# awkrail/svpc

Hardware: AMD Instinct MI355X
Metric: train steps/sec (vivt, batch=16, clip_seq=12) (higher is better)
Workload: dtype bf16x3

## Files before the change

### include/svpc_hip.h

```cpp
#ifndef SVPC_HIP_H
#define SVPC_HIP_H
#include <stddef.h>
#ifdef __cplusplus
extern "C" {
#endif

typedef struct ihipStream_t* svpc_stream_t;
typedef unsigned long long svpc_u64;

#define SVPC_ACT_NONE 0
#define SVPC_ACT_RELU 1
#define SVPC_ACT_GELU 2
#define SVPC_ACT_SIGMOID 3

const char* svpc_last_error(void);
int svpc_abi_version(void);

int svpc_ln_fwd(const float* x, const int* src_rows, const float* res, const float* gamma, const float* beta, float* y,
                float* mean, float* rstd, int R, int D, float eps, float p_pre, unsigned site_pre, float p_post,
                unsigned site_post, const svpc_u64* seed, const float* add1, int mod1, const float* add2, const int* idx2,
                svpc_stream_t stream);
int svpc_ln_fwd_t(const void* x, int x_dt, const int* src_rows, const void* res, const float* gamma, const float* beta, void* y,
                  int y_dt, float* mean, float* rstd, int R, int D, float eps, float p_pre, unsigned site_pre, float p_post,
                  unsigned site_post, const svpc_u64* seed, const float* add1, int mod1, const float* add2, const int* idx2,
// ... 8 lines not shown
int svpc_ln_param_grads(const float* partial, int R, int D, float* dgamma, float* dbeta, int accumulate, svpc_stream_t stream);
int svpc_ln_fwd_s(const void* x, int x_dt, int ldx, int lox, const int* src_rows, const void* res, int ldr, int lor, const float* gamma,
                  const float* beta, void* y, int y_dt, int ldy, int loy, float* mean, float* rstd, int R, int D, float eps, float p_pre,
                  unsigned site_pre, float p_post, unsigned site_post, const svpc_u64* seed, const float* add1, int mod1,
                  const float* add2, const int* idx2, svpc_stream_t stream);
int svpc_ln_bwd_rows_s(const void* dy, const void* x, int x_dt, int ldx, int y_dt, const int* src_rows, const void* res, int ldr,
                       const float* gamma, const float* mean, const float* rstd, void* dh, void* dx, float* partial, int R, int D,
                       float p_pre, unsigned site_pre, float p_post, unsigned site_post, const svpc_u64* seed, svpc_stream_t stream);
int svpc_bucket_colsum_t(const void* x, int x_dt, int ldx, const int* idx, int R, int C, int K, float* out, int accumulate,
                         float* workspace, svpc_stream_t stream);
typedef struct svpc_finalize_entry { const float* partial; float* out0; float* out1; int groups, ncols, split; } svpc_finalize_entry;
int svpc_colsum_partial_t(const void* x, int x_dt, int ldx, int R, int C, float* partial, svpc_stream_t stream);
typedef struct svpc_colsum_entry { const void* x; float* partial; int dt, ldx, R, C; } svpc_colsum_entry;
int svpc_multi_colsum(const svpc_colsum_entry* entries, int n, svpc_stream_t stream);
int svpc_multi_finalize_max(void);
int svpc_multi_finalize(const svpc_finalize_entry* entries, int n, svpc_stream_t stream);
int svpc_ln_bwd_groups(int R);
int svpc_ln_param_only_groups(int R);
int svpc_ln_param_grads_g(const float* partial, int groups, int D, float* dgamma, float* dbeta, int accumulate, svpc_stream_t stream);
int svpc_ln_bwd(const float* dy, const float* x, const int* src_rows, const float* res, const float* gamma,
                const float* mean, const float* rstd, float* dh, float* dx, float* dgamma, float* dbeta, int accumulate,
                float* workspace, int R, int D, float p_pre, unsigned site_pre, float p_post, unsigned site_post,
                const svpc_u64* seed, svpc_stream_t stream);
int svpc_colsum_chunks(int R);
int svpc_bucket_colsum(const float* x, int ldx, const int* idx, int R, int C, int K, float* out, int accumulate,
                       float* workspace, svpc_stream_t stream);

int svpc_gemm_f32(const float* A, int lda, int a_kc, const float* B, int ldb, int b_kc, float* C, int ldc, float* Z, int M, int N,
                  int K, const float* bias, int act, float p_drop, unsigned site, const svpc_u64* seed, int accumulate,
                  float* workspace, size_t workspace_bytes, svpc_stream_t stream);
int svpc_gemm_bf16(const float* A, int lda, int a_kc, const float* B, int ldb, int b_kc, float* C, int ldc, float* Z, int M, int N,
                   int K, const float* bias, int act, float p_drop, unsigned site, const svpc_u64* seed, int accumulate,
                   float* workspace, size_t workspace_bytes, svpc_stream_t stream);
int svpc_gemm_mx(const void* A, int a_dt, int lda, int a_kc, const void* B, int b_dt, int ldb, int b_kc, void* C, int c_dt, int ldc,
                 void* Z, int M, int N, int K, const float* bias, int act, float p_drop, unsigned site, const svpc_u64* seed,
                 int accumulate, float* workspace, size_t workspace_bytes, svpc_stream_t stream);
int svpc_gemm_glds_supported(int a_kc, int b_kc, int lda, int ldb, int M, int N, int K);
int svpc_gemm_glds(const void* A, int lda, int a_kc, const void* B, int ldb, int b_kc, void* C, int c_dt, int ldc, void* Z, int M, int N,
                   int K, const float* bias, int act, float p_drop, unsigned site, const svpc_u64* seed, int accumulate,
                   float* workspace, size_t workspace_bytes, svpc_stream_t stream);
int svpc_gemm_glds_r(const void* A, int lda, int a_kc, const void* B, int ldb, int b_kc, void* C, int c_dt, int ldc, void* Z, const void* R,
                     int M, int N, int K, const float* bias, int act, float p_drop, unsigned site, const svpc_u64* seed, int accumulate,
                     float* workspace, size_t workspace_bytes, svpc_stream_t stream);
int svpc_gemm_glds_rg(const void* A, int lda, int a_kc, const void* B, int ldb, int b_kc, void* C, int c_dt, int ldc, void* Z, const void* R,
                      const void* G, int gact, int M, int N, int K, const float* bias, int act, float p_drop, unsigned site,
                      const svpc_u64* seed, int accumulate, float* workspace, size_t workspace_bytes, svpc_stream_t stream);
int svpc_gemm_p8(const void* A, int lda, const void* B, int ldb, void* C, int ldc, void* Z, int M, int N, int K, const float* bias, int act,
                 svpc_stream_t stream);
int svpc_gemm_p8x3_supported(int lda, int a_lo, int ldb, int ldc, int c_lo, int ldz, int M, int N, int K);
int svpc_gemm_p8x3(const void* A, int lda, int a_lo, const void* B, int ldb, long long b_lo, void* C, int ldc, int c_lo, void* Z, int ldz,
                   int M, int N, int K, const float* bias, int act, svpc_stream_t stream);
int svpc_gemm_s4x3(const void* A, int lda, int a_lo, const void* B, int ldb, long long b_lo, void* C, int ldc, int c_lo, void* Z, int ldz,
                   int M, int N, int K, const float* bias, int act, svpc_stream_t stream);
int svpc_gemm_s4t_supported(int lda, int ldb, int ldc, int M, int N, int K);
int svpc_gemm_s4t(const void* A, int lda, const void* B, int ldb, void* C, int ldc, const void* R, int M, int N, int K, svpc_stream_t stream);
int svpc_gemm_p8t_supported(int lda, int ldb, int ldc, int M, int N, int K);
int svpc_gemm_p8t(const void* A, int lda, const void* B, int ldb, void* C, int ldc, const void* G, int gact, const void* R, int M, int N, int K,
                  svpc_stream_t stream);
int svpc_gemm_l32_supported(int a_kc, int b_kc, int lda, int ldb, int M, int N, int K);
int svpc_gemm_l32_preferred(int a_kc, int b_kc, int lda, int ldb, int M, int N, int K);
int svpc_gemm_l32(const float* A, int lda, int a_kc, const float* B, int ldb, int b_kc, float* C, int ldc, float* Z, int M, int N, int K,
                  const float* bias, int act, float p_drop, unsigned site, const svpc_u64* seed, int accumulate, float* workspace,
                  size_t workspace_bytes, svpc_stream_t stream);
int svpc_gemm_l32_r(const float* A, int lda, int a_kc, const float* B, int ldb, int b_kc, float* C, int ldc, float* Z, const float* R, int M,
                    int N, int K, const float* bias, int act, float p_drop, unsigned site, const svpc_u64* seed, int accumulate,
                    float* workspace, size_t workspace_bytes, svpc_stream_t stream);
int svpc_gemm_l32_rg(const float* A, int lda, int a_kc, const float* B, int ldb, int b_kc, float* C, int ldc, const float* R, const float* G,
                     int gact, int M, int N, int K, int accumulate, float* workspace, size_t workspace_bytes, svpc_stream_t stream);
int svpc_gemm_l32_x3(const float* A, int lda, int a_kc, const float* B, int ldb, int b_kc, float* C, int ldc, float* Z, const float* R, int M,
                     int N, int K, const float* bias, int act, float p_drop, unsigned site, const svpc_u64* seed, int accumulate,
                     float* workspace, size_t workspace_bytes, svpc_stream_t stream);
typedef struct svpc_gemm_problem { const float* A; const float* B; float* C; int M, N, K, lda, ldb, ldc; } svpc_gemm_problem;
int svpc_gemm_group(const svpc_gemm_problem* problems, int n, int a_kc, int b_kc, int accumulate, svpc_stream_t stream);
int svpc_gemm_group_x3(const svpc_gemm_problem* problems, int n, int a_kc, int b_kc, int accumulate, svpc_stream_t stream);
typedef struct svpc_wgrad_problem {
    const float* dz; const float* x; float* dw; float* db;
    int n_out, n_in, rows, ld_dz, ld_x, ld_dw;
} svpc_wgrad_problem;
int svpc_gemm_group_wgrad_max(void);
int svpc_gemm_group_wgrad_bf16_p8_ok(const void* problems, int n);
int svpc_gemm_group_wgrad_bf16_p8(const void* problems, int n, float* workspace, size_t workspace_bytes, svpc_stream_t stream);
int svpc_gemm_group_wgrad_bf16(const svpc_wgrad_problem* problems, int n, svpc_stream_t stream);
int svpc_gemm_group_wgrad_bf16_ws(const svpc_wgrad_problem* problems, int n, float* workspace, size_t workspace_bytes,
                                  svpc_stream_t stream);
int svpc_gemm_group_wgrad(const svpc_wgrad_problem* problems, int n, svpc_stream_t stream);
int svpc_act_bwd(const float* dy, const float* aux, float* dz, size_t n, int act, float p, unsigned site, const svpc_u64* seed,
                 svpc_stream_t stream);

int svpc_act_bwd_t(const void* dy, const void* aux, void* dz, int dt, size_t n, int act, float p, unsigned site, const svpc_u64* seed,
                   svpc_stream_t stream);

int svpc_attn_fwd(const float* Q, int ldq, const float* K, int ldk, const float* V, int ldv, float* O, int ldo, float* LSE,
                  const int* seq, int n_seq, int H, int dh, int max_q, int max_k, const float* key_mask, int causal, float scale,
                  float p_drop, unsigned site, const svpc_u64* seed, svpc_stream_t stream);
int svpc_attn_q1_fwd(const float* Q, int ldq, const float* K, int ldk, const float* V, int ldv, float* O, int ldo, float* LSE,
                     const int* seq, int n_seq, int H, int dh, int max_k, const float* key_mask, float scale, svpc_stream_t stream);
int svpc_attn_q1_ln_supported(int D, int dh, int n_keys, int ldq, int ldkv, int ldnew, int ldx, int ldo);
int svpc_attn_q1_ln_fwd(const float* Q, int ldq, float* K, float* V, int ldkv, int k_stride, int n_keys, const float* newK, const float* newV,
                        int ldnew, const float* X, int ldx, const float* gamma, const float* beta, float eps, float* O, int ldo, int T, int D,
                        int dh, float scale, svpc_stream_t stream);
int svpc_attn_q1_ln_idx_fwd(const float* Q, int ldq, float* K, float* V, int ldkv, int k_stride, int n_keys, const int* key_rows, int ld_rows,
                            int q_group, const float* newK, const float* newV, int ldnew, const float* X, int ldx, const float* gamma,
                            const float* beta, float eps, float* O, int ldo, int T, int D, int dh, float scale, svpc_stream_t stream);
int svpc_attn_bwd(const float* Q, int ldq, const float* K, int ldk, const float* V, int ldv, const float* O, int ldo,
                  const float* LSE, const float* dO, int lddo, float* dQ, int lddq, float* dK, int lddk, float* dV, int lddv,
                  float* delta, const int* seq, int n_seq, int H, int dh, int max_q, int max_k, const float* key_mask, int causal,
                  float scale, float p_drop, unsigned site, const svpc_u64* seed, svpc_stream_t stream);

// ... 202 lines not shown
```

### svpc_amd/csrc/gemm_common.h

```cpp
#pragma once
#include "common.h"

typedef float floatx16 __attribute__((ext_vector_type(16)));

struct Epi {
    const float* bias; int act; float p_drop; uint32_t site; const u64* seed; int accumulate;
    float* Z;
    const void* R;
    const void* G; int gact;
};

__device__ __forceinline__ void epilogue_store(float v, int row, int col, float* __restrict__ C, int ldc, const Epi& e,
                                               u64 seed, float inv_keep) {
    if (e.bias) v += e.bias[col];
    const size_t o = (size_t)row * ldc + col;
    if (e.Z) e.Z[o] = v;
    v = apply_act(v, e.act);
    if (e.p_drop > 0.f) v *= drop_scale(seed, e.site, o, e.p_drop, inv_keep);
    if (e.G) v *= act_grad_from_aux(reinterpret_cast<const float*>(e.G)[o], e.gact, false);
    if (e.accumulate) v += C[o];
    if (e.R) v += reinterpret_cast<const float*>(e.R)[o];
    C[o] = v;
}

// ... 67 lines not shown
    return (xcd < r ? xcd * (q + 1) : r * (q + 1) + (xcd - r) * q) + (orig >> 3);
}


template <typename TC>
__global__ __launch_bounds__(256) void splitk_reduce1_kernel(const float* __restrict__ slabs, int splitk, TC* __restrict__ C, int ldc,
                                                             int M, int N, Epi epi) {
    const size_t i = (size_t)blockIdx.x * 256 + threadIdx.x;
    if (i >= (size_t)M * N) return;
    const int row = (int)(i / N), col = (int)(i - (size_t)row * N);
    float s = 0.f;
    for (int k = 0; k < splitk; ++k) s += slabs[(size_t)k * M * N + i];
    const u64 seed = epi.p_drop > 0.f ? epi.seed[0] : 0ull;
    const float inv_keep = epi.p_drop > 0.f ? 1.0f / (1.0f - epi.p_drop) : 1.0f;
    epilogue_store_t<TC>(s, row, col, C, ldc, epi, seed, inv_keep);
}
template <typename TC>
__global__ __launch_bounds__(256) void splitk_reduce4_kernel(const float* __restrict__ slabs, int splitk, TC* __restrict__ C, int ldc,
                                                             int M, int N, Epi epi) {
    const size_t q = (size_t)blockIdx.x * 256 + threadIdx.x, nq = (size_t)M * N / 4;
    if (q >= nq) return;
    const size_t i = q * 4;
    const int row = (int)(i / N), col = (int)(i - (size_t)row * N);
    const float4* p = reinterpret_cast<const float4*>(slabs) + q;
    float4 s = make_float4(0.f, 0.f, 0.f, 0.f);
    int k = 0;
    for (; k + 4 <= splitk; k += 4) {
        const float4 a = p[(size_t)k * nq], b = p[(size_t)(k + 1) * nq], c = p[(size_t)(k + 2) * nq], d = p[(size_t)(k + 3) * nq];
        s.x += a.x; s.y += a.y; s.z += a.z; s.w += a.w;
        s.x += b.x; s.y += b.y; s.z += b.z; s.w += b.w;
        s.x += c.x; s.y += c.y; s.z += c.z; s.w += c.w;
        s.x += d.x; s.y += d.y; s.z += d.z; s.w += d.w;
    }
    for (; k < splitk; ++k) {
        const float4 a = p[(size_t)k * nq];
        s.x += a.x; s.y += a.y; s.z += a.z; s.w += a.w;
    }
    const u64 seed = epi.p_drop > 0.f ? epi.seed[0] : 0ull;
    const float inv_keep = epi.p_drop > 0.f ? 1.0f / (1.0f - epi.p_drop) : 1.0f;
    epilogue_store_t<TC>(s.x, row, col, C, ldc, epi, seed, inv_keep);
    epilogue_store_t<TC>(s.y, row, col + 1, C, ldc, epi, seed, inv_keep);
    epilogue_store_t<TC>(s.z, row, col + 2, C, ldc, epi, seed, inv_keep);
    epilogue_store_t<TC>(s.w, row, col + 3, C, ldc, epi, seed, inv_keep);
}
template <typename TC>
static inline void launch_splitk_reduce(const float* slabs, int splitk, TC* C, int ldc, int M, int N, const Epi& epi, hipStream_t stream) {
    const size_t n = (size_t)M * N;
    if (N % 4 == 0 && ((((uintptr_t)slabs) & 15) == 0))
        hipLaunchKernelGGL(splitk_reduce4_kernel<TC>, dim3((unsigned)((n / 4 + 255) / 256)), dim3(256), 0, stream, slabs, splitk, C, ldc, M, N,
                           epi);
    else
        hipLaunchKernelGGL(splitk_reduce1_kernel<TC>, dim3((unsigned)((n + 255) / 256)), dim3(256), 0, stream, slabs, splitk, C, ldc, M, N, epi);
}
```

### svpc_amd/csrc/gemm_s4t.hip

```cpp
#include "gemm_common.h"
#include <stdlib.h>

typedef __bf16 bf16x8 __attribute__((ext_vector_type(8)));
typedef float floatx4 __attribute__((ext_vector_type(4)));
typedef short short4s __attribute__((ext_vector_type(4)));
typedef const void __attribute__((address_space(1))) * s4t_gptr;
typedef void __attribute__((address_space(3))) * s4t_lptr;

constexpr int S4T_BK = 64;
constexpr int S4T_HALF = 128 * S4T_BK * 2;
constexpr int S4T_STAGE = 2 * S4T_HALF;

__device__ __forceinline__ bf16x8 s4t_frag_tr(const char* __restrict__ a) {
    typedef short4s __attribute__((address_space(3))) * lds_ptr;
    const short4s lo = __builtin_amdgcn_ds_read_tr16_b64_v4i16((lds_ptr)(a));
    const short4s hi = __builtin_amdgcn_ds_read_tr16_b64_v4i16((lds_ptr)(a + 4 * 256));
    union { short s[8]; bf16x8 v; } u;
    u.s[0] = lo[0]; u.s[1] = lo[1]; u.s[2] = lo[2]; u.s[3] = lo[3];
    u.s[4] = hi[0]; u.s[5] = hi[1]; u.s[6] = hi[2]; u.s[7] = hi[3];
    return u.v;
}

template <bool HASR, int NS>
__global__ __launch_bounds__(512, NS == 2 ? 2 : 1) void gemm_s4t_kernel(const __bf16* __restrict__ A, int lda, const __bf16* __restrict__ B, int ldb,
                                                                        __bf16* __restrict__ C, int ldc, const __bf16* __restrict__ R, int M,
                                                                        int N, int K, int tiles_m, int tiles_n, int remap) {
    __shared__ __attribute__((aligned(1024))) char smem[NS * S4T_STAGE];
    const int wg = remap ? xcd_remap(blockIdx.x, tiles_m * tiles_n) : (int)blockIdx.x;
    const int tm = wg / tiles_n, tn = wg - tm * tiles_n;
    const int m0 = tm * 128, n0 = tn * 128;
    const int nk = K / S4T_BK;
    const int lane = threadIdx.x & 63, wave = __builtin_amdgcn_readfirstlane(threadIdx.x >> 6);
    const int wr = wave >> 1, wc = wave & 1;

    const int sr = lane >> 2, sc = (lane & 3) ^ (((lane >> 5) & 1) << 1);
    const __bf16* const ga = A + (size_t)min(m0 + 16 * wave + sr, M - 1) * lda + 8 * sc;
    const __bf16* gb[2];
#pragma unroll
    for (int u = 0; u < 2; ++u) {
        const int kr = 8 * wave + 4 * u + (lane >> 4);
        const int fx = 2 * ((kr & 3) | ((kr >> 1) & 4));
        const int col = min(n0 + 8 * ((lane & 15) ^ fx), N - 8);
        gb[u] = B + (size_t)kr * ldb + col;
    }
    const size_t stepB = (size_t)S4T_BK * ldb;
#define S4T_ISSUE(t)                                                                                                              \
    do {                                                                                                                          \
        char* st_ = smem + ((t) % NS) * S4T_STAGE;                                                                                \
        const __bf16* sa_ = ga + (size_t)(t) * S4T_BK;                                                                            \
        __builtin_amdgcn_global_load_lds((s4t_gptr)(sa_), (s4t_lptr)(st_ + ((wave * 2) << 10)), 16, 0, 0);                        \
        __builtin_amdgcn_global_load_lds((s4t_gptr)(sa_ + 32), (s4t_lptr)(st_ + ((wave * 2 + 1) << 10)), 16, 0, 0);               \
        __builtin_amdgcn_global_load_lds((s4t_gptr)(gb[0] + (size_t)(t) * stepB), (s4t_lptr)(st_ + S4T_HALF + wave * 2048), 16, 0, 0);        \
        __builtin_amdgcn_global_load_lds((s4t_gptr)(gb[1] + (size_t)(t) * stepB), (s4t_lptr)(st_ + S4T_HALF + wave * 2048 + 1024), 16, 0, 0); \
    } while (0)
    const int fr_off = (lane & 15) * 64 + ((((lane >> 4) ^ (((lane >> 3) & 1) << 1))) << 4);
#define S4T_FRAGA(img, blk, kb) (*reinterpret_cast<const bf16x8*>((img) + (((blk) * 2 + (kb)) << 10) + fr_off))
    const int tg = lane >> 4, tq = (lane & 15) >> 2, tp = lane & 3;
    const int tfx = 2 * (tq + 4 * (tg & 1));
    const int tb_off = (8 * tg + tq) * 256 + ((tp & 1) << 3);
    const int tp1 = tp >> 1;
#define S4T_FRAGB(img, cb, kb) s4t_frag_tr((img) + (kb) * (32 * 256) + tb_off + (((((2 * (cb)) ^ tfx)) | tp1) << 4))

    floatx4 acc[2][4];
#pragma unroll
    for (int i = 0; i < 2; ++i)
#pragma unroll
        for (int j = 0; j < 4; ++j) acc[i][j] = floatx4{0.f, 0.f, 0.f, 0.f};

#pragma unroll
    for (int t = 0; t < NS - 1; ++t)
        if (t < nk) S4T_ISSUE(t);
    for (int t = 0; t < nk; ++t) {
        if (NS == 4 && t + 2 < nk) asm volatile("s_waitcnt vmcnt(8)" ::: "memory");
        else if (NS >= 3 && t + 1 < nk) asm volatile("s_waitcnt vmcnt(4)" ::: "memory");
        else asm volatile("s_waitcnt vmcnt(0)" ::: "memory");
        __builtin_amdgcn_s_barrier();
        __builtin_amdgcn_sched_barrier(0);
        if (t + NS - 1 < nk) S4T_ISSUE(t + NS - 1);
        const char* sa = smem + (t % NS) * S4T_STAGE;
        const char* sb = sa + S4T_HALF;
#pragma unroll
        for (int kb = 0; kb < 2; ++kb) {
            bf16x8 bfr[4], afr[2];
#pragma unroll
            for (int j = 0; j < 4; ++j) bfr[j] = S4T_FRAGB(sb, wc * 4 + j, kb);
#pragma unroll
            for (int i = 0; i < 2; ++i) afr[i] = S4T_FRAGA(sa, wr * 2 + i, kb);
#pragma unroll
            for (int i = 0; i < 2; ++i)
#pragma unroll
                for (int j = 0; j < 4; ++j) acc[i][j] = __builtin_amdgcn_mfma_f32_16x16x32_bf16(bfr[j], afr[i], acc[i][j], 0, 0, 0);
        }
    }
#undef S4T_ISSUE
#undef S4T_FRAGA
#undef S4T_FRAGB
    __syncthreads();
    char* wl = smem + wave * 8192;
    const int row0 = m0 + wr * 32, col0 = n0 + wc * 64;
    const int l15 = lane & 15, q = lane >> 4;
    const int c8 = lane & 7, cc = col0 + 8 * c8, r0 = lane >> 3;
    const bool col_ok = cc + 8 <= N;
    bf16x8 rv[HASR ? 4 : 1];
#pragma unroll
    for (int it = 0; it < 4; ++it) {
        const int r = it * 8 + r0;
        if (HASR && col_ok && row0 + r < M) rv[it] = *reinterpret_cast<const bf16x8*>(R + (size_t)(row0 + r) * ldc + cc);
    }
#pragma unroll
    for (int i = 0; i < 2; ++i) {
        const int r = i * 16 + l15;
#pragma unroll
        for (int j = 0; j < 4; ++j) {
            const int c16 = j * 4 + q;
            *reinterpret_cast<floatx4*>(wl + r * 256 + ((c16 ^ (r & 7)) << 4)) = acc[i][j];
        }
    }
#pragma unroll
    for (int it = 0; it < 4; ++it) {
        const int r = it * 8 + r0;
        const floatx4 v0 = *reinterpret_cast<const floatx4*>(wl + r * 256 + (((2 * c8) ^ (r & 7)) << 4));
        const floatx4 v1 = *reinterpret_cast<const floatx4*>(wl + r * 256 + (((2 * c8 + 1) ^ (r & 7)) << 4));
        float v[8] = {v0[0], v0[1], v0[2], v0[3], v1[0], v1[1], v1[2], v1[3]};
        if (col_ok && row0 + r < M) {
            const size_t o = (size_t)(row0 + r) * ldc + cc;
            if (HASR) {
#pragma unroll
                for (int j = 0; j < 8; ++j) v[j] += (float)rv[it][j];
            }
            bf16x8 ov;
#pragma unroll
            for (int j = 0; j < 8; ++j) ov[j] = (__bf16)v[j];
            *reinterpret_cast<bf16x8*>(C + o) = ov;
        }
    }
}

extern "C" {

int svpc_gemm_s4t_supported(int lda, int ldb, int ldc, int M, int N, int K) {
    if (M <= 0 || N < 8 || K < S4T_BK || K % S4T_BK != 0 || (N & 7) != 0) return 0;
    if ((lda & 7) || (ldb & 7) || (ldc & 7) || lda < K || ldb < N || ldc < N) return 0;
    return 1;
}

int svpc_gemm_s4t(const void* A, int lda, const void* B, int ldb, void* C, int ldc, const void* R, int M, int N, int K, hipStream_t stream) {
    if (M <= 0 || N <= 0) return 0;
    SVPC_REQUIRE(svpc_gemm_s4t_supported(lda, ldb, ldc, M, N, K) == 1 &&
                     ((((uintptr_t)A) | ((uintptr_t)B) | ((uintptr_t)C) | ((uintptr_t)R)) & 15) == 0,
                 "gemm_s4t: needs K % 64 == 0, N % 8 == 0, 16-byte aligned bf16 rows");
    static int remap = -1, deep_max = -1;
    if (remap < 0) { const char* e = getenv("SVPC_GEMM_REMAP"); remap = e ? atoi(e) : 1; }
    if (deep_max < 0) { const char* e = getenv("SVPC_S4T_DEEP_MAX"); deep_max = e ? atoi(e) : 256; }
    const int tiles_m = ceil_div(M, 128), tiles_n = ceil_div(N, 128);
    const bool deep = tiles_m * tiles_n <= deep_max;
#define S4T_GO(RV, NSV)                                                                                                           \
    hipLaunchKernelGGL((gemm_s4t_kernel<RV, NSV>), dim3(tiles_m * tiles_n), dim3(512), 0, stream, (const __bf16*)A, lda, (const __bf16*)B, \
                       ldb, (__bf16*)C, ldc, (const __bf16*)R, M, N, K, tiles_m, tiles_n, remap)
    if (R != nullptr) { if (deep) S4T_GO(true, 4); else S4T_GO(true, 2); }
    else { if (deep) S4T_GO(false, 4); else S4T_GO(false, 2); }
#undef S4T_GO
    return svpc_check_launch("gemm_s4t");
}

}
```

### svpc_amd/csrc/gemm_s4x3.hip

```cpp
#include "gemm_common.h"
#include <stdlib.h>

typedef __bf16 bf16x8 __attribute__((ext_vector_type(8)));
typedef float floatx4 __attribute__((ext_vector_type(4)));
typedef const void __attribute__((address_space(1))) * s4_gptr;
typedef void __attribute__((address_space(3))) * s4_lptr;

constexpr int S4_BK = 64;
constexpr int S4_KS = 32;
constexpr int S4_HALF = 128 * S4_BK * 2;
constexpr int S4_STAGE = 2 * S4_HALF;

__device__ __forceinline__ uint32_t s4_pack2(float lo, float hi) {
    union { __bf16 h[2]; uint32_t u; } pk;
    pk.h[0] = (__bf16)lo; pk.h[1] = (__bf16)hi;
    return pk.u;
}
__device__ __forceinline__ float s4_lo(float v) { return v - (float)(__bf16)v; }
__device__ __forceinline__ float s4_gelu(float x) {
    const float u = x * 0.70710678118654752f, au = fabsf(u);
    const float t = __builtin_amdgcn_rcpf(fmaf(0.3275911f, au, 1.0f));
    float p = fmaf(1.061405429f, t, -1.453152027f);
    p = fmaf(p, t, 1.421413741f);
    p = fmaf(p, t, -0.284496736f);
    p = fmaf(p, t, 0.254829592f);
    const float e = __expf(-au * au);
    return 0.5f * x * (1.0f + copysignf(fmaf(-p * t, e, 1.0f), u));
}
template <int ACT>
__device__ __forceinline__ float s4_act(float z) {
    if (ACT == ACT_RELU) return fmaxf(z, 0.f);
    if (ACT == ACT_GELU) return s4_gelu(z);
    return z;
}

template <int ACT, int MODE>
__device__ __forceinline__ void s4_store_pass(const floatx4 (&acc)[2][4], __bf16* __restrict__ C, int ldc, const float4 (&bb)[4], int row0,
                                              int col0, int M, int N, int lane, char* __restrict__ wl) {
    const int l15 = lane & 15, q = lane >> 4;
#pragma unroll
    for (int i = 0; i < 2; ++i) {
        const int r = i * 16 + l15;
#pragma unroll
        for (int j = 0; j < 4; ++j) {
            float z0 = acc[i][j][0] + bb[j].x, z1 = acc[i][j][1] + bb[j].y, z2 = acc[i][j][2] + bb[j].z, z3 = acc[i][j][3] + bb[j].w;
            if (MODE != 0) { z0 = s4_act<ACT>(z0); z1 = s4_act<ACT>(z1); z2 = s4_act<ACT>(z2); z3 = s4_act<ACT>(z3); }
            if (MODE == 2) { z0 = s4_lo(z0); z1 = s4_lo(z1); z2 = s4_lo(z2); z3 = s4_lo(z3); }
            uint2 v;
            v.x = s4_pack2(z0, z1); v.y = s4_pack2(z2, z3);
            const int c16 = j * 2 + (q >> 1);
            *reinterpret_cast<uint2*>(wl + r * 128 + ((c16 ^ (r & 7)) << 4) + ((q & 1) << 3)) = v;
        }
    }
    const int chunk = lane & 7, cc = col0 + 8 * chunk, r0 = lane >> 3;
    uint32_t off = ((uint32_t)(row0 + r0) * (uint32_t)ldc + (uint32_t)cc) * 2u;
    const uint32_t step = 16u * (uint32_t)ldc;
    const bool col_ok = cc + 8 <= N;
#pragma unroll
    for (int it = 0; it < 4; ++it) {
        const int r = it * 8 + r0;
        const uint4 v = *reinterpret_cast<const uint4*>(wl + r * 128 + ((chunk ^ (r & 7)) << 4));
        if (col_ok && row0 + r < M) *reinterpret_cast<uint4*>(reinterpret_cast<char*>(C) + off) = v;
        off += step;
    }
}

template <int ACT, bool HASZ, int NS>
__global__ __launch_bounds__(512, NS == 2 ? 2 : 1) void gemm_s4x3_kernel(const __bf16* __restrict__ A, int lda, int a_lo, const __bf16* __restrict__ B, int ldb,
                                                           long long b_lo, __bf16* __restrict__ C, int ldc, int c_lo, __bf16* __restrict__ Z,
                                                           int ldz, const float* __restrict__ bias, int M, int N, int K, int tiles_m,
                                                           int tiles_n, int remap) {
    __shared__ __attribute__((aligned(1024))) char smem[NS * S4_STAGE];
    const int wg = remap ? xcd_remap(blockIdx.x, tiles_m * tiles_n) : (int)blockIdx.x;
    const int tm = wg / tiles_n, tn = wg - tm * tiles_n;
    const int m0 = tm * 128, n0 = tn * 128;
    const int nk = K / S4_KS;
    const int lane = threadIdx.x & 63, wave = __builtin_amdgcn_readfirstlane(threadIdx.x >> 6);
    const int wr = wave >> 1, wc = wave & 1;

    const int sr = lane >> 2, sc = (lane & 3) ^ (((lane >> 5) & 1) << 1);
    const __bf16* const ga = A + (size_t)min(m0 + 16 * wave + sr, M - 1) * lda + 8 * sc;
    const __bf16* const gb = B + (size_t)min(n0 + 16 * wave + sr, N - 1) * ldb + 8 * sc;
#define S4_ISSUE(t)                                                                                                               \
    do {                                                                                                                          \
        char* da_ = smem + ((t) % NS) * S4_STAGE + ((wave * 2) << 10);                                                            \
        const size_t o_ = (size_t)(t) * S4_KS;                                                                                    \
        __builtin_amdgcn_global_load_lds((s4_gptr)(ga + o_), (s4_lptr)(da_), 16, 0, 0);                                           \
        __builtin_amdgcn_global_load_lds((s4_gptr)(ga + o_ + a_lo), (s4_lptr)(da_ + 1024), 16, 0, 0);                             \
        __builtin_amdgcn_global_load_lds((s4_gptr)(gb + o_), (s4_lptr)(da_ + S4_HALF), 16, 0, 0);                                 \
        __builtin_amdgcn_global_load_lds((s4_gptr)(gb + o_ + b_lo), (s4_lptr)(da_ + S4_HALF + 1024), 16, 0, 0);                   \
    } while (0)
    const int fr_off = (lane & 15) * 64 + ((((lane >> 4) ^ (((lane >> 3) & 1) << 1))) << 4);
#define S4_FRAG(img, blk, kb) (*reinterpret_cast<const bf16x8*>((img) + (((blk) * 2 + (kb)) << 10) + fr_off))

    floatx4 acc[2][4];
#pragma unroll
    for (int i = 0; i < 2; ++i)
#pragma unroll
        for (int j = 0; j < 4; ++j) acc[i][j] = floatx4{0.f, 0.f, 0.f, 0.f};

#pragma unroll
    for (int t = 0; t < NS - 1; ++t)
        if (t < nk) S4_ISSUE(t);
    for (int t = 0; t < nk; ++t) {
        if (NS == 4 && t + 2 < nk) asm volatile("s_waitcnt vmcnt(8)" ::: "memory");
        else if (NS >= 3 && t + 1 < nk) asm volatile("s_waitcnt vmcnt(4)" ::: "memory");
        else asm volatile("s_waitcnt vmcnt(0)" ::: "memory");
        __builtin_amdgcn_s_barrier();
        __builtin_amdgcn_sched_barrier(0);
        if (t + NS - 1 < nk) S4_ISSUE(t + NS - 1);
        const char* sa = smem + (t % NS) * S4_STAGE;
        const char* sb = sa + S4_HALF;
        bf16x8 bfr[2][4], afr[2][2];
#pragma unroll
        for (int pl = 0; pl < 2; ++pl) {
#pragma unroll
            for (int j = 0; j < 4; ++j) bfr[pl][j] = S4_FRAG(sb, wc * 4 + j, pl);
#pragma unroll
            for (int i = 0; i < 2; ++i) afr[pl][i] = S4_FRAG(sa, wr * 2 + i, pl);
        }
#pragma unroll
        for (int term = 0; term < 3; ++term)
#pragma unroll
            for (int i = 0; i < 2; ++i)
#pragma unroll
                for (int j = 0; j < 4; ++j)
                    acc[i][j] = __builtin_amdgcn_mfma_f32_16x16x32_bf16(bfr[term == 2 ? 1 : 0][j], afr[term == 0 ? 1 : 0][i], acc[i][j], 0, 0, 0);
    }
#undef S4_ISSUE
#undef S4_FRAG
    __syncthreads();
    char* wl = smem + wave * 4096;
    const int row0 = m0 + wr * 32, col0 = n0 + wc * 64;
    float4 bb[4];
#pragma unroll
    for (int j = 0; j < 4; ++j) {
        const int c = col0 + j * 16 + 4 * (lane >> 4);
        bb[j] = (bias && c + 4 <= N) ? *reinterpret_cast<const float4*>(bias + c) : make_float4(0.f, 0.f, 0.f, 0.f);
    }
    if (HASZ) s4_store_pass<ACT, 0>(acc, Z, ldz, bb, row0, col0, M, N, lane, wl);
    s4_store_pass<ACT, 2>(acc, C + c_lo, ldc, bb, row0, col0, M, N, lane, wl);
    s4_store_pass<ACT, 1>(acc, C, ldc, bb, row0, col0, M, N, lane, wl);
}

extern "C" {

int svpc_gemm_s4x3(const void* A, int lda, int a_lo, const void* B, int ldb, long long b_lo, void* C, int ldc, int c_lo, void* Z, int ldz,
                   int M, int N, int K, const float* bias, int act, hipStream_t stream) {
    if (M <= 0 || N <= 0) return 0;
    if (Z == nullptr) ldz = 0;
    SVPC_REQUIRE(K >= 2 * S4_KS && K % S4_KS == 0 && (N & 7) == 0 && !((lda | a_lo | ldb | ldc | c_lo | ldz) & 7) && a_lo >= K && lda >= a_lo + K &&
                     c_lo >= N && ldc >= c_lo + N && ldb >= K && (b_lo & 7) == 0 &&
                     (unsigned long long)M * (unsigned long long)ldc * 2ull < (1ull << 32) &&
                     ((((uintptr_t)A) | ((uintptr_t)B) | ((uintptr_t)C) | ((uintptr_t)Z) | ((uintptr_t)bias)) & 15) == 0 &&
                     (act == ACT_RELU || act == ACT_GELU || (act == ACT_NONE && Z == nullptr)) && (Z == nullptr || ldz >= N),
                 "gemm_s4x3: needs K % 32 == 0, K >= 64, N % 8 == 0, 16-byte aligned split rows (lo plane behind the hi plane), act in {none, relu, gelu}");
    static int remap = -1;
    if (remap < 0) { const char* e = getenv("SVPC_GEMM_REMAP"); remap = e ? atoi(e) : 1; }
    const int tiles_m = ceil_div(M, 128), tiles_n = ceil_div(N, 128);
    static int deep_max = -1;
    if (deep_max < 0) { const char* e = getenv("SVPC_S4X3_DEEP_MAX"); deep_max = e ? atoi(e) : 256; }
    const bool deep = tiles_m * tiles_n <= deep_max;
#define S4_GO(ACTV, ZV)                                                                                                           \
    do {                                                                                                                          \
        if (deep) hipLaunchKernelGGL((gemm_s4x3_kernel<ACTV, ZV, 4>), dim3(tiles_m * tiles_n), dim3(512), 0, stream, (const __bf16*)A, lda, a_lo, \
                       (const __bf16*)B, ldb, b_lo, (__bf16*)C, ldc, c_lo, (__bf16*)Z, ldz, bias, M, N, K, tiles_m, tiles_n, remap); \
        else hipLaunchKernelGGL((gemm_s4x3_kernel<ACTV, ZV, 2>), dim3(tiles_m * tiles_n), dim3(512), 0, stream, (const __bf16*)A, lda, a_lo, \
                       (const __bf16*)B, ldb, b_lo, (__bf16*)C, ldc, c_lo, (__bf16*)Z, ldz, bias, M, N, K, tiles_m, tiles_n, remap); \
    } while (0)
    const bool z = Z != nullptr;
    if (act == ACT_GELU) { if (z) S4_GO(ACT_GELU, true); else S4_GO(ACT_GELU, false); }
    else if (act == ACT_RELU) { if (z) S4_GO(ACT_RELU, true); else S4_GO(ACT_RELU, false); }
    else S4_GO(ACT_NONE, false);
#undef S4_GO
    return svpc_check_launch("gemm_s4x3");
}

}
```

Before: 91.06.

## Add 96/192 tile variants to split-bf16 GEMMs with CU-aware tile picker

Templates the s4x3 and s4t GEMM kernels on tile size, adding 96 (and 192 for s4x3) geometries with matching wave layouts, LDS swizzles and store passes. A host picker estimates wave count times tile depth against the CU count and picks 96 when it gives fewer waves of work than 128. The aim is to cut tail-wave underuse on shapes whose 128-tile count fits the CU count poorly. The cost is smaller tiles with less operand reuse, plus a new non-power-of-two B swizzle that is a correctness risk.

```diff
diff --git a/include/svpc_hip.h b/include/svpc_hip.h
--- a/include/svpc_hip.h
+++ b/include/svpc_hip.h
@@ -84,8 +84,13 @@
                    int M, int N, int K, const float* bias, int act, svpc_stream_t stream);
 int svpc_gemm_s4x3(const void* A, int lda, int a_lo, const void* B, int ldb, long long b_lo, void* C, int ldc, int c_lo, void* Z, int ldz,
                    int M, int N, int K, const float* bias, int act, svpc_stream_t stream);
+int svpc_gemm_s4x3_tile(const void* A, int lda, int a_lo, const void* B, int ldb, long long b_lo, void* C, int ldc, int c_lo, void* Z, int ldz,
+                        int M, int N, int K, const float* bias, int act, int tile, svpc_stream_t stream);
+int svpc_gemm_s4_pick_tile(int M, int N, int cus);
 int svpc_gemm_s4t_supported(int lda, int ldb, int ldc, int M, int N, int K);
 int svpc_gemm_s4t(const void* A, int lda, const void* B, int ldb, void* C, int ldc, const void* R, int M, int N, int K, svpc_stream_t stream);
+int svpc_gemm_s4t_tile(const void* A, int lda, const void* B, int ldb, void* C, int ldc, const void* R, int M, int N, int K, int tile,
+                       svpc_stream_t stream);
 int svpc_gemm_p8t_supported(int lda, int ldb, int ldc, int M, int N, int K);
 int svpc_gemm_p8t(const void* A, int lda, const void* B, int ldb, void* C, int ldc, const void* G, int gact, const void* R, int M, int N, int K,
                   svpc_stream_t stream);
diff --git a/svpc_amd/csrc/gemm_common.h b/svpc_amd/csrc/gemm_common.h
--- a/svpc_amd/csrc/gemm_common.h
+++ b/svpc_amd/csrc/gemm_common.h
@@ -143,3 +143,15 @@
     else
         hipLaunchKernelGGL(splitk_reduce1_kernel<TC>, dim3((unsigned)((n + 255) / 256)), dim3(256), 0, stream, slabs, splitk, C, ldc, M, N, epi);
 }
+
+
+static inline int s4_tile_cost(int bt, int M, int N, int cus) { return ceil_div(ceil_div(M, bt) * ceil_div(N, bt), cus) * 2 * bt; }
+static inline int s4_pick_tile(int M, int N, int cus) { return s4_tile_cost(96, M, N, cus) < s4_tile_cost(128, M, N, cus) ? 96 : 128; }
+static inline int s4_cu_count() {
+    static int cus = -1;
+    if (cus < 0) {
+        hipDeviceProp_t prop; int dev = 0;
+        cus = (hipGetDevice(&dev) == hipSuccess && hipGetDeviceProperties(&prop, dev) == hipSuccess) ? prop.multiProcessorCount : 256;
+    }
+    return cus;
+}
diff --git a/svpc_amd/csrc/gemm_s4t.hip b/svpc_amd/csrc/gemm_s4t.hip
--- a/svpc_amd/csrc/gemm_s4t.hip
+++ b/svpc_amd/csrc/gemm_s4t.hip
@@ -8,64 +8,82 @@
 typedef void __attribute__((address_space(3))) * s4t_lptr;
 
 constexpr int S4T_BK = 64;
-constexpr int S4T_HALF = 128 * S4T_BK * 2;
-constexpr int S4T_STAGE = 2 * S4T_HALF;
 
+template <int BT> struct S4tGeo;
+template <> struct S4tGeo<96> { static constexpr int WR = 3, WC = 2, TI = 2, TJ = 3; };
+template <> struct S4tGeo<128> { static constexpr int WR = 4, WC = 2, TI = 2, TJ = 4; };
+
+template <int ROWB>
 __device__ __forceinline__ bf16x8 s4t_frag_tr(const char* __restrict__ a) {
     typedef short4s __attribute__((address_space(3))) * lds_ptr;
     const short4s lo = __builtin_amdgcn_ds_read_tr16_b64_v4i16((lds_ptr)(a));
-    const short4s hi = __builtin_amdgcn_ds_read_tr16_b64_v4i16((lds_ptr)(a + 4 * 256));
+    const short4s hi = __builtin_amdgcn_ds_read_tr16_b64_v4i16((lds_ptr)(a + 4 * ROWB));
     union { short s[8]; bf16x8 v; } u;
     u.s[0] = lo[0]; u.s[1] = lo[1]; u.s[2] = lo[2]; u.s[3] = lo[3];
     u.s[4] = hi[0]; u.s[5] = hi[1]; u.s[6] = hi[2]; u.s[7] = hi[3];
     return u.v;
 }
 
-template <bool HASR, int NS>
-__global__ __launch_bounds__(512, NS == 2 ? 2 : 1) void gemm_s4t_kernel(const __bf16* __restrict__ A, int lda, const __bf16* __restrict__ B, int ldb,
+template <bool HASR, int NS, int BT>
+__global__ __launch_bounds__(BT * 4, NS == 2 ? 2 : 1) void gemm_s4t_kernel(const __bf16* __restrict__ A, int lda, const __bf16* __restrict__ B, int ldb,
                                                                         __bf16* __restrict__ C, int ldc, const __bf16* __restrict__ R, int M,
                                                                         int N, int K, int tiles_m, int tiles_n, int remap) {
-    __shared__ __attribute__((aligned(1024))) char smem[NS * S4T_STAGE];
+    typedef S4tGeo<BT> G;
+    constexpr int TI = G::TI, TJ = G::TJ;
+    static_assert(G::WR * G::WC * 16 == BT && G::WR * TI * 16 == BT && G::WC * TJ * 16 == BT && TI == 2, "s4t geometry");
+    constexpr int ROWB = BT * 2;
+    constexpr int HALF_A = BT * S4T_BK * 2, STAGE = HALF_A + S4T_BK * ROWB;
+    static_assert(NS * STAGE <= 160 * 1024 && G::WR * G::WC * 8192 <= NS * STAGE, "s4t LDS");
+    __shared__ __attribute__((aligned(1024))) char smem[NS * STAGE];
     const int wg = remap ? xcd_remap(blockIdx.x, tiles_m * tiles_n) : (int)blockIdx.x;
     const int tm = wg / tiles_n, tn = wg - tm * tiles_n;
-    const int m0 = tm * 128, n0 = tn * 128;
+    const int m0 = tm * BT, n0 = tn * BT;
     const int nk = K / S4T_BK;
     const int lane = threadIdx.x & 63, wave = __builtin_amdgcn_readfirstlane(threadIdx.x >> 6);
-    const int wr = wave >> 1, wc = wave & 1;
+    const int wr = wave / G::WC, wc = wave - wr * G::WC;
 
     const int sr = lane >> 2, sc = (lane & 3) ^ (((lane >> 5) & 1) << 1);
     const __bf16* const ga = A + (size_t)min(m0 + 16 * wave + sr, M - 1) * lda + 8 * sc;
     const __bf16* gb[2];
 #pragma unroll
     for (int u = 0; u < 2; ++u) {
-        const int kr = 8 * wave + 4 * u + (lane >> 4);
-        const int fx = 2 * ((kr & 3) | ((kr >> 1) & 4));
-        const int col = min(n0 + 8 * ((lane & 15) ^ fx), N - 8);
+        int kr, ch;
+        if (BT == 128) {
+            kr = 8 * wave + 4 * u + (lane >> 4);
+            ch = (lane & 15) ^ (2 * ((kr & 3) | ((kr >> 1) & 4)));
+        } else {
+            const int s = 64 * (2 * wave + u) + lane;
+            kr = s / 12;
+            ch = s - 12 * kr - 2 * ((kr >> 3) & 1);
+            if (ch < 0) ch += 12;
+        }
+        const int col = min(n0 + 8 * ch, N - 8);
         gb[u] = B + (size_t)kr * ldb + col;
     }
     const size_t stepB = (size_t)S4T_BK * ldb;
 #define S4T_ISSUE(t)                                                                                                              \
     do {                                                                                                                          \
-        char* st_ = smem + ((t) % NS) * S4T_STAGE;                                                                                \
+        char* st_ = smem + ((t) % NS) * STAGE;                                                                                    \
         const __bf16* sa_ = ga + (size_t)(t) * S4T_BK;                                                                            \
         __builtin_amdgcn_global_load_lds((s4t_gptr)(sa_), (s4t_lptr)(st_ + ((wave * 2) << 10)), 16, 0, 0);                        \
         __builtin_amdgcn_global_load_lds((s4t_gptr)(sa_ + 32), (s4t_lptr)(st_ + ((wave * 2 + 1) << 10)), 16, 0, 0);               \
-        __builtin_amdgcn_global_load_lds((s4t_gptr)(gb[0] + (size_t)(t) * stepB), (s4t_lptr)(st_ + S4T_HALF + wave * 2048), 16, 0, 0);        \
-        __builtin_amdgcn_global_load_lds((s4t_gptr)(gb[1] + (size_t)(t) * stepB), (s4t_lptr)(st_ + S4T_HALF + wave * 2048 + 1024), 16, 0, 0); \
+        __builtin_amdgcn_global_load_lds((s4t_gptr)(gb[0] + (size_t)(t) * stepB), (s4t_lptr)(st_ + HALF_A + wave * 2048), 16, 0, 0);          \
+        __builtin_amdgcn_global_load_lds((s4t_gptr)(gb[1] + (size_t)(t) * stepB), (s4t_lptr)(st_ + HALF_A + wave * 2048 + 1024), 16, 0, 0);   \
     } while (0)
     const int fr_off = (lane & 15) * 64 + ((((lane >> 4) ^ (((lane >> 3) & 1) << 1))) << 4);
 #define S4T_FRAGA(img, blk, kb) (*reinterpret_cast<const bf16x8*>((img) + (((blk) * 2 + (kb)) << 10) + fr_off))
     const int tg = lane >> 4, tq = (lane & 15) >> 2, tp = lane & 3;
-    const int tfx = 2 * (tq + 4 * (tg & 1));
-    const int tb_off = (8 * tg + tq) * 256 + ((tp & 1) << 3);
+    const int tfx = BT == 128 ? 2 * (tq + 4 * (tg & 1)) : 2 * (tg & 1);
+    const int tb_off = (8 * tg + tq) * ROWB + ((tp & 1) << 3);
     const int tp1 = tp >> 1;
-#define S4T_FRAGB(img, cb, kb) s4t_frag_tr((img) + (kb) * (32 * 256) + tb_off + (((((2 * (cb)) ^ tfx)) | tp1) << 4))
+#define S4T_SLOT(cb) (BT == 128 ? (((2 * (cb)) ^ tfx) | tp1) : ((2 * (cb) + tfx >= 12 ? 2 * (cb) + tfx - 12 : 2 * (cb) + tfx) | tp1))
+#define S4T_FRAGB(img, cb, kb) s4t_frag_tr<ROWB>((img) + (kb) * (32 * ROWB) + tb_off + (S4T_SLOT(cb) << 4))
 
-    floatx4 acc[2][4];
+    floatx4 acc[TI][TJ];
 #pragma unroll
-    for (int i = 0; i < 2; ++i)
+    for (int i = 0; i < TI; ++i)
 #pragma unroll
-        for (int j = 0; j < 4; ++j) acc[i][j] = floatx4{0.f, 0.f, 0.f, 0.f};
+        for (int j = 0; j < TJ; ++j) acc[i][j] = floatx4{0.f, 0.f, 0.f, 0.f};
 
 #pragma unroll
     for (int t = 0; t < NS - 1; ++t)
@@ -77,30 +95,31 @@
         __builtin_amdgcn_s_barrier();
         __builtin_amdgcn_sched_barrier(0);
         if (t + NS - 1 < nk) S4T_ISSUE(t + NS - 1);
-        const char* sa = smem + (t % NS) * S4T_STAGE;
-        const char* sb = sa + S4T_HALF;
+        const char* sa = smem + (t % NS) * STAGE;
+        const char* sb = sa + HALF_A;
 #pragma unroll
         for (int kb = 0; kb < 2; ++kb) {
-            bf16x8 bfr[4], afr[2];
+            bf16x8 bfr[TJ], afr[TI];
 #pragma unroll
-            for (int j = 0; j < 4; ++j) bfr[j] = S4T_FRAGB(sb, wc * 4 + j, kb);
+            for (int j = 0; j < TJ; ++j) bfr[j] = S4T_FRAGB(sb, wc * TJ + j, kb);
 #pragma unroll
-            for (int i = 0; i < 2; ++i) afr[i] = S4T_FRAGA(sa, wr * 2 + i, kb);
+            for (int i = 0; i < TI; ++i) afr[i] = S4T_FRAGA(sa, wr * TI + i, kb);
 #pragma unroll
-            for (int i = 0; i < 2; ++i)
+            for (int i = 0; i < TI; ++i)
 #pragma unroll
-                for (int j = 0; j < 4; ++j) acc[i][j] = __builtin_amdgcn_mfma_f32_16x16x32_bf16(bfr[j], afr[i], acc[i][j], 0, 0, 0);
+                for (int j = 0; j < TJ; ++j) acc[i][j] = __builtin_amdgcn_mfma_f32_16x16x32_bf16(bfr[j], afr[i], acc[i][j], 0, 0, 0);
         }
     }
 #undef S4T_ISSUE
 #undef S4T_FRAGA
 #undef S4T_FRAGB
+#undef S4T_SLOT
     __syncthreads();
     char* wl = smem + wave * 8192;
-    const int row0 = m0 + wr * 32, col0 = n0 + wc * 64;
+    const int row0 = m0 + wr * 32, col0 = n0 + wc * TJ * 16;
     const int l15 = lane & 15, q = lane >> 4;
     const int c8 = lane & 7, cc = col0 + 8 * c8, r0 = lane >> 3;
-    const bool col_ok = cc + 8 <= N;
+    const bool col_ok = c8 < 2 * TJ && cc + 8 <= N;
     bf16x8 rv[HASR ? 4 : 1];
 #pragma unroll
     for (int it = 0; it < 4; ++it) {
@@ -108,10 +127,10 @@
         if (HASR && col_ok && row0 + r < M) rv[it] = *reinterpret_cast<const bf16x8*>(R + (size_t)(row0 + r) * ldc + cc);
     }
 #pragma unroll
-    for (int i = 0; i < 2; ++i) {
+    for (int i = 0; i < TI; ++i) {
         const int r = i * 16 + l15;
 #pragma unroll
-        for (int j = 0; j < 4; ++j) {
+        for (int j = 0; j < TJ; ++j) {
             const int c16 = j * 4 + q;
             *reinterpret_cast<floatx4*>(wl + r * 256 + ((c16 ^ (r & 7)) << 4)) = acc[i][j];
         }
@@ -144,23 +163,36 @@
     return 1;
 }
 
-int svpc_gemm_s4t(const void* A, int lda, const void* B, int ldb, void* C, int ldc, const void* R, int M, int N, int K, hipStream_t stream) {
+int svpc_gemm_s4t_tile(const void* A, int lda, const void* B, int ldb, void* C, int ldc, const void* R, int M, int N, int K, int tile,
+                       hipStream_t stream) {
     if (M <= 0 || N <= 0) return 0;
     SVPC_REQUIRE(svpc_gemm_s4t_supported(lda, ldb, ldc, M, N, K) == 1 &&
                      ((((uintptr_t)A) | ((uintptr_t)B) | ((uintptr_t)C) | ((uintptr_t)R)) & 15) == 0,
                  "gemm_s4t: needs K % 64 == 0, N % 8 == 0, 16-byte aligned bf16 rows");
+    SVPC_REQUIRE(tile == 0 || tile == 96 || tile == 128, "gemm_s4t: tile must be 0 (pick), 96 or 128");
     static int remap = -1, deep_max = -1;
     if (remap < 0) { const char* e = getenv("SVPC_GEMM_REMAP"); remap = e ? atoi(e) : 1; }
     if (deep_max < 0) { const char* e = getenv("SVPC_S4T_DEEP_MAX"); deep_max = e ? atoi(e) : 256; }
-    const int tiles_m = ceil_div(M, 128), tiles_n = ceil_div(N, 128);
+    const int bt = tile ? tile : s4_pick_tile(M, N, s4_cu_count());
+    const int tiles_m = ceil_div(M, bt), tiles_n = ceil_div(N, bt);
     const bool deep = tiles_m * tiles_n <= deep_max;
-#define S4T_GO(RV, NSV)                                                                                                           \
-    hipLaunchKernelGGL((gemm_s4t_kernel<RV, NSV>), dim3(tiles_m * tiles_n), dim3(512), 0, stream, (const __bf16*)A, lda, (const __bf16*)B, \
-                       ldb, (__bf16*)C, ldc, (const __bf16*)R, M, N, K, tiles_m, tiles_n, remap)
-    if (R != nullptr) { if (deep) S4T_GO(true, 4); else S4T_GO(true, 2); }
-    else { if (deep) S4T_GO(false, 4); else S4T_GO(false, 2); }
+#define S4T_LAUNCH(RV, NSV, BTV)                                                                                                  \
+    hipLaunchKernelGGL((gemm_s4t_kernel<RV, NSV, BTV>), dim3(tiles_m * tiles_n), dim3(BTV * 4), 0, stream, (const __bf16*)A, lda,   \
+                       (const __bf16*)B, ldb, (__bf16*)C, ldc, (const __bf16*)R, M, N, K, tiles_m, tiles_n, remap)
+#define S4T_GO(RV)                                                                                                                \
+    do {                                                                                                                          \
+        if (bt == 96) { if (deep) S4T_LAUNCH(RV, 4, 96); else S4T_LAUNCH(RV, 2, 96); }                                            \
+        else { if (deep) S4T_LAUNCH(RV, 4, 128); else S4T_LAUNCH(RV, 2, 128); }                                                   \
+    } while (0)
+    if (R != nullptr) S4T_GO(true);
+    else S4T_GO(false);
 #undef S4T_GO
+#undef S4T_LAUNCH
     return svpc_check_launch("gemm_s4t");
 }
 
+int svpc_gemm_s4t(const void* A, int lda, const void* B, int ldb, void* C, int ldc, const void* R, int M, int N, int K, hipStream_t stream) {
+    return svpc_gemm_s4t_tile(A, lda, B, ldb, C, ldc, R, M, N, K, 0, stream);
 }
+
+}
diff --git a/svpc_amd/csrc/gemm_s4x3.hip b/svpc_amd/csrc/gemm_s4x3.hip
--- a/svpc_amd/csrc/gemm_s4x3.hip
+++ b/svpc_amd/csrc/gemm_s4x3.hip
@@ -8,8 +8,11 @@
 
 constexpr int S4_BK = 64;
 constexpr int S4_KS = 32;
-constexpr int S4_HALF = 128 * S4_BK * 2;
-constexpr int S4_STAGE = 2 * S4_HALF;
+
+template <int BT> struct S4Geo;
+template <> struct S4Geo<96> { static constexpr int WR = 3, WC = 2, TI = 2, TJ = 3; };
+template <> struct S4Geo<128> { static constexpr int WR = 4, WC = 2, TI = 2, TJ = 4; };
+template <> struct S4Geo<192> { static constexpr int WR = 4, WC = 3, TI = 3, TJ = 4; };
 
 __device__ __forceinline__ uint32_t s4_pack2(float lo, float hi) {
     union { __bf16 h[2]; uint32_t u; } pk;
@@ -34,15 +37,15 @@
     return z;
 }
 
-template <int ACT, int MODE>
-__device__ __forceinline__ void s4_store_pass(const floatx4 (&acc)[2][4], __bf16* __restrict__ C, int ldc, const float4 (&bb)[4], int row0,
+template <int ACT, int MODE, int TI, int TJ>
+__device__ __forceinline__ void s4_store_pass(const floatx4 (&acc)[TI][TJ], __bf16* __restrict__ C, int ldc, const float4 (&bb)[TJ], int row0,
                                               int col0, int M, int N, int lane, char* __restrict__ wl) {
     const int l15 = lane & 15, q = lane >> 4;
 #pragma unroll
-    for (int i = 0; i < 2; ++i) {
+    for (int i = 0; i < TI; ++i) {
         const int r = i * 16 + l15;
 #pragma unroll
-        for (int j = 0; j < 4; ++j) {
+        for (int j = 0; j < TJ; ++j) {
             float z0 = acc[i][j][0] + bb[j].x, z1 = acc[i][j][1] + bb[j].y, z2 = acc[i][j][2] + bb[j].z, z3 = acc[i][j][3] + bb[j].w;
             if (MODE != 0) { z0 = s4_act<ACT>(z0); z1 = s4_act<ACT>(z1); z2 = s4_act<ACT>(z2); z3 = s4_act<ACT>(z3); }
             if (MODE == 2) { z0 = s4_lo(z0); z1 = s4_lo(z1); z2 = s4_lo(z2); z3 = s4_lo(z3); }
@@ -55,9 +58,9 @@
     const int chunk = lane & 7, cc = col0 + 8 * chunk, r0 = lane >> 3;
     uint32_t off = ((uint32_t)(row0 + r0) * (uint32_t)ldc + (uint32_t)cc) * 2u;
     const uint32_t step = 16u * (uint32_t)ldc;
-    const bool col_ok = cc + 8 <= N;
-#pragma unroll
-    for (int it = 0; it < 4; ++it) {
+    const bool col_ok = chunk < 2 * TJ && cc + 8 <= N;
+#pragma unroll
+    for (int it = 0; it < 2 * TI; ++it) {
         const int r = it * 8 + r0;
         const uint4 v = *reinterpret_cast<const uint4*>(wl + r * 128 + ((chunk ^ (r & 7)) << 4));
         if (col_ok && row0 + r < M) *reinterpret_cast<uint4*>(reinterpret_cast<char*>(C) + off) = v;
@@ -65,39 +68,44 @@
     }
 }
 
-template <int ACT, bool HASZ, int NS>
-__global__ __launch_bounds__(512, NS == 2 ? 2 : 1) void gemm_s4x3_kernel(const __bf16* __restrict__ A, int lda, int a_lo, const __bf16* __restrict__ B, int ldb,
+template <int ACT, bool HASZ, int NS, int BT>
+__global__ __launch_bounds__(BT * 4, NS == 2 ? 2 : 1) void gemm_s4x3_kernel(const __bf16* __restrict__ A, int lda, int a_lo, const __bf16* __restrict__ B, int ldb,
                                                            long long b_lo, __bf16* __restrict__ C, int ldc, int c_lo, __bf16* __restrict__ Z,
                                                            int ldz, const float* __restrict__ bias, int M, int N, int K, int tiles_m,
                                                            int tiles_n, int remap) {
-    __shared__ __attribute__((aligned(1024))) char smem[NS * S4_STAGE];
+    typedef S4Geo<BT> G;
+    constexpr int TI = G::TI, TJ = G::TJ;
+    static_assert(G::WR * G::WC * 16 == BT && G::WR * TI * 16 == BT && G::WC * TJ * 16 == BT, "s4x3 geometry");
+    constexpr int HALF = BT * S4_BK * 2, STAGE = 2 * HALF;
+    static_assert(NS * STAGE <= 160 * 1024 && G::WR * G::WC * TI * 16 * 128 <= NS * STAGE, "s4x3 LDS");
+    __shared__ __attribute__((aligned(1024))) char smem[NS * STAGE];
     const int wg = remap ? xcd_remap(blockIdx.x, tiles_m * tiles_n) : (int)blockIdx.x;
     const int tm = wg / tiles_n, tn = wg - tm * tiles_n;
-    const int m0 = tm * 128, n0 = tn * 128;
+    const int m0 = tm * BT, n0 = tn * BT;
     const int nk = K / S4_KS;
     const int lane = threadIdx.x & 63, wave = __builtin_amdgcn_readfirstlane(threadIdx.x >> 6);
-    const int wr = wave >> 1, wc = wave & 1;
+    const int wr = wave / G::WC, wc = wave - wr * G::WC;
 
     const int sr = lane >> 2, sc = (lane & 3) ^ (((lane >> 5) & 1) << 1);
     const __bf16* const ga = A + (size_t)min(m0 + 16 * wave + sr, M - 1) * lda + 8 * sc;
     const __bf16* const gb = B + (size_t)min(n0 + 16 * wave + sr, N - 1) * ldb + 8 * sc;
 #define S4_ISSUE(t)                                                                                                               \
     do {                                                                                                                          \
-        char* da_ = smem + ((t) % NS) * S4_STAGE + ((wave * 2) << 10);                                                            \
+        char* da_ = smem + ((t) % NS) * STAGE + ((wave * 2) << 10);                                                               \
         const size_t o_ = (size_t)(t) * S4_KS;                                                                                    \
         __builtin_amdgcn_global_load_lds((s4_gptr)(ga + o_), (s4_lptr)(da_), 16, 0, 0);                                           \
         __builtin_amdgcn_global_load_lds((s4_gptr)(ga + o_ + a_lo), (s4_lptr)(da_ + 1024), 16, 0, 0);                             \
-        __builtin_amdgcn_global_load_lds((s4_gptr)(gb + o_), (s4_lptr)(da_ + S4_HALF), 16, 0, 0);                                 \
-        __builtin_amdgcn_global_load_lds((s4_gptr)(gb + o_ + b_lo), (s4_lptr)(da_ + S4_HALF + 1024), 16, 0, 0);                   \
+        __builtin_amdgcn_global_load_lds((s4_gptr)(gb + o_), (s4_lptr)(da_ + HALF), 16, 0, 0);                                    \
+        __builtin_amdgcn_global_load_lds((s4_gptr)(gb + o_ + b_lo), (s4_lptr)(da_ + HALF + 1024), 16, 0, 0);                      \
     } while (0)
     const int fr_off = (lane & 15) * 64 + ((((lane >> 4) ^ (((lane >> 3) & 1) << 1))) << 4);
 #define S4_FRAG(img, blk, kb) (*reinterpret_cast<const bf16x8*>((img) + (((blk) * 2 + (kb)) << 10) + fr_off))
 
-    floatx4 acc[2][4];
-#pragma unroll
-    for (int i = 0; i < 2; ++i)
-#pragma unroll
-        for (int j = 0; j < 4; ++j) acc[i][j] = floatx4{0.f, 0.f, 0.f, 0.f};
+    floatx4 acc[TI][TJ];
+#pragma unroll
+    for (int i = 0; i < TI; ++i)
+#pragma unroll
+        for (int j = 0; j < TJ; ++j) acc[i][j] = floatx4{0.f, 0.f, 0.f, 0.f};
 
 #pragma unroll
     for (int t = 0; t < NS - 1; ++t)
@@ -109,44 +117,49 @@
         __builtin_amdgcn_s_barrier();
         __builtin_amdgcn_sched_barrier(0);
         if (t + NS - 1 < nk) S4_ISSUE(t + NS - 1);
-        const char* sa = smem + (t % NS) * S4_STAGE;
-        const char* sb = sa + S4_HALF;
-        bf16x8 bfr[2][4], afr[2][2];
+        const char* sa = smem + (t % NS) * STAGE;
+        const char* sb = sa + HALF;
+        bf16x8 bfr[2][TJ], afr[2][TI];
 #pragma unroll
         for (int pl = 0; pl < 2; ++pl) {
 #pragma unroll
-            for (int j = 0; j < 4; ++j) bfr[pl][j] = S4_FRAG(sb, wc * 4 + j, pl);
-#pragma unroll
-            for (int i = 0; i < 2; ++i) afr[pl][i] = S4_FRAG(sa, wr * 2 + i, pl);
+            for (int j = 0; j < TJ; ++j) bfr[pl][j] = S4_FRAG(sb, wc * TJ + j, pl);
+#pragma unroll
+            for (int i = 0; i < TI; ++i) afr[pl][i] = S4_FRAG(sa, wr * TI + i, pl);
         }
 #pragma unroll
         for (int term = 0; term < 3; ++term)
 #pragma unroll
-            for (int i = 0; i < 2; ++i)
-#pragma unroll
-                for (int j = 0; j < 4; ++j)
+            for (int i = 0; i < TI; ++i)
+#pragma unroll
+                for (int j = 0; j < TJ; ++j)
                     acc[i][j] = __builtin_amdgcn_mfma_f32_16x16x32_bf16(bfr[term == 2 ? 1 : 0][j], afr[term == 0 ? 1 : 0][i], acc[i][j], 0, 0, 0);
     }
 #undef S4_ISSUE
 #undef S4_FRAG
     __syncthreads();
-    char* wl = smem + wave * 4096;
-    const int row0 = m0 + wr * 32, col0 = n0 + wc * 64;
-    float4 bb[4];
-#pragma unroll
-    for (int j = 0; j < 4; ++j) {
+    char* wl = smem + wave * (TI * 16 * 128);
+    const int row0 = m0 + wr * TI * 16, col0 = n0 + wc * TJ * 16;
+    float4 bb[TJ];
+#pragma unroll
+    for (int j = 0; j < TJ; ++j) {
         const int c = col0 + j * 16 + 4 * (lane >> 4);
         bb[j] = (bias && c + 4 <= N) ? *reinterpret_cast<const float4*>(bias + c) : make_float4(0.f, 0.f, 0.f, 0.f);
     }
-    if (HASZ) s4_store_pass<ACT, 0>(acc, Z, ldz, bb, row0, col0, M, N, lane, wl);
-    s4_store_pass<ACT, 2>(acc, C + c_lo, ldc, bb, row0, col0, M, N, lane, wl);
-    s4_store_pass<ACT, 1>(acc, C, ldc, bb, row0, col0, M, N, lane, wl);
+    if (HASZ) s4_store_pass<ACT, 0, TI, TJ>(acc, Z, ldz, bb, row0, col0, M, N, lane, wl);
+    s4_store_pass<ACT, 2, TI, TJ>(acc, C + c_lo, ldc, bb, row0, col0, M, N, lane, wl);
+    s4_store_pass<ACT, 1, TI, TJ>(acc, C, ldc, bb, row0, col0, M, N, lane, wl);
 }
 
 extern "C" {
 
-int svpc_gemm_s4x3(const void* A, int lda, int a_lo, const void* B, int ldb, long long b_lo, void* C, int ldc, int c_lo, void* Z, int ldz,
-                   int M, int N, int K, const float* bias, int act, hipStream_t stream) {
+int svpc_gemm_s4_pick_tile(int M, int N, int cus) {
+    if (M <= 0 || N <= 0 || cus <= 0) return 128;
+    return s4_pick_tile(M, N, cus);
+}
+
+int svpc_gemm_s4x3_tile(const void* A, int lda, int a_lo, const void* B, int ldb, long long b_lo, void* C, int ldc, int c_lo, void* Z, int ldz,
+                        int M, int N, int K, const float* bias, int act, int tile, hipStream_t stream) {
     if (M <= 0 || N <= 0) return 0;
     if (Z == nullptr) ldz = 0;
     SVPC_REQUIRE(K >= 2 * S4_KS && K % S4_KS == 0 && (N & 7) == 0 && !((lda | a_lo | ldb | ldc | c_lo | ldz) & 7) && a_lo >= K && lda >= a_lo + K &&
@@ -155,25 +168,35 @@
                      ((((uintptr_t)A) | ((uintptr_t)B) | ((uintptr_t)C) | ((uintptr_t)Z) | ((uintptr_t)bias)) & 15) == 0 &&
                      (act == ACT_RELU || act == ACT_GELU || (act == ACT_NONE && Z == nullptr)) && (Z == nullptr || ldz >= N),
                  "gemm_s4x3: needs K % 32 == 0, K >= 64, N % 8 == 0, 16-byte aligned split rows (lo plane behind the hi plane), act in {none, relu, gelu}");
+    SVPC_REQUIRE(tile == 0 || tile == 96 || tile == 128 || tile == 192, "gemm_s4x3: tile must be 0 (pick), 96, 128 or 192");
     static int remap = -1;
     if (remap < 0) { const char* e = getenv("SVPC_GEMM_REMAP"); remap = e ? atoi(e) : 1; }
-    const int tiles_m = ceil_div(M, 128), tiles_n = ceil_div(N, 128);
+    const int bt = tile ? tile : s4_pick_tile(M, N, s4_cu_count());
+    const int tiles_m = ceil_div(M, bt), tiles_n = ceil_div(N, bt);
     static int deep_max = -1;
     if (deep_max < 0) { const char* e = getenv("SVPC_S4X3_DEEP_MAX"); deep_max = e ? atoi(e) : 256; }
     const bool deep = tiles_m * tiles_n <= deep_max;
+#define S4_LAUNCH(ACTV, ZV, NSV, BTV)                                                                                             \
+    hipLaunchKernelGGL((gemm_s4x3_kernel<ACTV, ZV, NSV, BTV>), dim3(tiles_m * tiles_n), dim3(BTV * 4), 0, stream, (const __bf16*)A, lda, \
+                       a_lo, (const __bf16*)B, ldb, b_lo, (__bf16*)C, ldc, c_lo, (__bf16*)Z, ldz, bias, M, N, K, tiles_m, tiles_n, remap)
 #define S4_GO(ACTV, ZV)                                                                                                           \
     do {                                                                                                                          \
-        if (deep) hipLaunchKernelGGL((gemm_s4x3_kernel<ACTV, ZV, 4>), dim3(tiles_m * tiles_n), dim3(512), 0, stream, (const __bf16*)A, lda, a_lo, \
-                       (const __bf16*)B, ldb, b_lo, (__bf16*)C, ldc, c_lo, (__bf16*)Z, ldz, bias, M, N, K, tiles_m, tiles_n, remap); \
-        else hipLaunchKernelGGL((gemm_s4x3_kernel<ACTV, ZV, 2>), dim3(tiles_m * tiles_n), dim3(512), 0, stream, (const __bf16*)A, lda, a_lo, \
-                       (const __bf16*)B, ldb, b_lo, (__bf16*)C, ldc, c_lo, (__bf16*)Z, ldz, bias, M, N, K, tiles_m, tiles_n, remap); \
+        if (bt == 192) S4_LAUNCH(ACTV, ZV, 3, 192);                                                                               \
+        else if (bt == 96) { if (deep) S4_LAUNCH(ACTV, ZV, 4, 96); else S4_LAUNCH(ACTV, ZV, 2, 96); }                             \
+        else { if (deep) S4_LAUNCH(ACTV, ZV, 4, 128); else S4_LAUNCH(ACTV, ZV, 2, 128); }                                         \
     } while (0)
     const bool z = Z != nullptr;
     if (act == ACT_GELU) { if (z) S4_GO(ACT_GELU, true); else S4_GO(ACT_GELU, false); }
     else if (act == ACT_RELU) { if (z) S4_GO(ACT_RELU, true); else S4_GO(ACT_RELU, false); }
     else S4_GO(ACT_NONE, false);
 #undef S4_GO
+#undef S4_LAUNCH
     return svpc_check_launch("gemm_s4x3");
 }
 
-}
+int svpc_gemm_s4x3(const void* A, int lda, int a_lo, const void* B, int ldb, long long b_lo, void* C, int ldc, int c_lo, void* Z, int ldz,
+                   int M, int N, int K, const float* bias, int act, hipStream_t stream) {
+    return svpc_gemm_s4x3_tile(A, lda, a_lo, B, ldb, b_lo, C, ldc, c_lo, Z, ldz, M, N, K, bias, act, 0, stream);
+}
+
+}
```

Result: no change. 91.64, median of 6 (+0.6%).
